# prestodb/presto

Measured on AMD Instinct MI355X. Metric: tpch_lineitem_rows_per_sec, higher is better.
Workload: dtype f64; 1 GPU; TPC-H SF100 Q1 & Q3 on 1xMI355X - one step = one Q1 pass + one Q3 pass, columns resident in HBM; query=q1+q3, rows_per_gpu=1200075804, mode=f64

## Files before the change

include/presto_gpu.h:

```cpp
#ifndef PRESTO_GPU_H
#define PRESTO_GPU_H
#include <stdint.h>

#ifdef __cplusplus
extern "C" {
#endif

#define PG_ABI_VERSION 1

typedef int32_t pg_status;
#define PG_OK 0
#define PG_ERR (-1)
const char* pg_last_error(void);

pg_status pg_device_count(int32_t* out);
pg_status pg_device_sync(void);
pg_status pg_device_malloc(int64_t bytes, void** out);
pg_status pg_device_free(void* p);
pg_status pg_memcpy_h2d(void* dst, const void* src, int64_t bytes);
pg_status pg_memcpy_d2h(void* dst, const void* src, int64_t bytes);
pg_status pg_memcpy_d2d(void* dst, const void* src, int64_t bytes);
double pg_last_hot_kernel_ms(void);
double pg_hot_max_ms(void);
void pg_hot_reset(void);
// ... 217 lines not shown
typedef enum { PG_WIN_ROW_NUMBER = 0, PG_WIN_RANK, PG_WIN_DENSE_RANK,
               PG_WIN_COUNT, PG_WIN_SUM, PG_WIN_MIN, PG_WIN_MAX,
               PG_WIN_LAG, PG_WIN_LEAD } pg_win_func;
typedef enum { PG_FRAME_RANGE_RUNNING = 0,
               PG_FRAME_ROWS_RUNNING  = 1,
               PG_FRAME_PARTITION     = 2   } pg_win_frame;
typedef struct { int32_t func;
                 int32_t col;
                 int32_t frame;
                 int32_t pad;
                 int64_t offset;
} pg_win_spec;

typedef struct {
    int32_t n_keys;
    int32_t n_partition_keys;
    int32_t key_col[PG_MAX_SORT_KEYS];
    int32_t order[PG_MAX_SORT_KEYS];
    int32_t n_emit;
    int32_t emit_cols[PG_MAX_SORT_EMIT];
    int32_t n_funcs;
    pg_win_spec funcs[PG_MAX_WIN_FUNCS];
} pg_plan_window;

#define PG_DISTINCT_MARK 0
#define PG_DISTINCT_ONLY 1

typedef struct {
    int64_t capacity_hint;
    int64_t limit;
    int32_t n_keys;
    int32_t key_col[4];
    int32_t mode;
    int32_t n_emit;
    int32_t emit_cols[16];
} pg_plan_mark_distinct;

typedef int64_t pg_op;

pg_status pg_op_create(int32_t kind, const void* plan, int64_t plan_bytes,
                       pg_op* out);
int32_t pg_op_needs_input(pg_op op);
pg_status pg_op_add_input(pg_op op, const pg_page* page);
pg_status pg_op_get_output(pg_op op, const pg_page** out);
pg_status pg_op_finish(pg_op op);
int32_t pg_op_is_finished(pg_op op);
pg_status pg_op_destroy(pg_op op);

pg_status pg_op_table(pg_op op, int64_t* out_table);
pg_status pg_op_partition_counts(pg_op op, int64_t* counts, int32_t n);

pg_status pg_table_destroy(int64_t table);
pg_status pg_table_reset_acc(int64_t table);

pg_status pg_page_serialize(const pg_page* page ,
                            void* out, int64_t cap, int64_t* out_len);
int32_t pg_abi_struct_sizes(int32_t* out, int32_t n);
int32_t pg_abi_plan_size(int32_t kind);
uint64_t pg_sortkey_u64(int32_t tag, int32_t order, uint64_t bits);

pg_status pg_page_serialize2(const pg_page* page, int32_t compress,
                             void* out, int64_t cap, int64_t* out_len);
pg_status pg_page_deserialize(const void* buf, int64_t len, pg_page* out);
pg_status pg_page_free(pg_page* page);

#ifdef __cplusplus
}
#endif
#endif
```

presto_amd/csrc/kernels.hip:

```cpp
#include <hip/hip_runtime.h>
#include <stdio.h>
#include <stdlib.h>
#include <string.h>
#include <map>
#include <vector>
#include <algorithm>
#include <type_traits>
#include <stdexcept>
#include <string>

#include "../../include/presto_gpu.h"
#include "fixed128.h"
#include "sortkey.h"

static __thread char g_err[512];
extern "C" const char* pg_last_error(void) { return g_err; }
static pg_status seterr(const char* msg)
{
    snprintf(g_err, sizeof(g_err), "%s", msg);
    return PG_ERR;
}
#define CHK(x)                                                          \
    do {                                                                \
        hipError_t e_ = (x);                                            \
// ... 1266 lines not shown
        int64_t s = (int64_t)(h & (uint64_t)mask);
        int64_t tries = 0;
        for (;;) {
            int64_t old = atomicCAS((unsigned long long*)&keys[s],
                                    (unsigned long long)TBL_EMPTY,
                                    (unsigned long long)word);
            if (old == TBL_EMPTY || old == word) {
                if (old == TBL_EMPTY) {
                    my_inserted++;
                    if (tags) tags[s] = d_tbl_tag(h);
                }
                if (pbits) break;
                if (lu_payload && dp.n >= 1)
                    ((uint8_t*)dp.ptr[0])[s] = plv;
                for (int o = lu_payload ? 1 : 0; o < dp.n; o++) {
                    const pg_col& c = pg.cols[dp.src[o]];
                    switch (dp.tag[o]) {
                        case PG_T_U8:
                            ((uint8_t*)dp.ptr[o])[s] =
                                (uint8_t)d_load_i64(c, i);
                            break;
                        case PG_T_I32:
                            ((int32_t*)dp.ptr[o])[s] =
                                (int32_t)d_load_i64(c, i);
                            break;
                        case PG_T_I64:
                            ((int64_t*)dp.ptr[o])[s] = d_load_i64(c, i);
                            break;
                        default:
                            ((double*)dp.ptr[o])[s] = d_load_f64(c, i);
                    }
                }
                break;
            }
            if (++tries > mask) {
                my_overflow++;
                break;
            }
            s = (s + 1) & mask;
        }
    }
    my_inserted = d_bfly_i64(my_inserted);
    my_overflow = d_bfly_i64(my_overflow);
    my_packerr = d_bfly_i64(my_packerr);
    if ((threadIdx.x & 63) == 0) {
        if (my_inserted) atomicAdd(inserted, (unsigned long long)my_inserted);
        if (my_overflow) atomicAdd(overflow, (unsigned long long)my_overflow);
        if (my_packerr) atomicAdd(pack_err, (unsigned long long)my_packerr);
    }
}

#define BS_R 4
#define BS_TILE (256 * BS_R)
struct staged_args {
    const int32_t* pc[2];
    int64_t pval[2];
    int32_t pop[2];
    int32_t n_preds;
    const int64_t* sk;
    const uint8_t* flags;
    int64_t nflags;
    const int64_t* lk;
    const uint8_t* lu;
    int64_t lucap;
    const int64_t* key;
    const void* pay;
    int32_t pay_tag;
    int32_t pay_pred;
    int64_t n;
};
__device__ inline bool d_cmp_i64(int32_t op, int64_t v, int64_t x)
{
    switch (op) {
        case PG_CMP_LT: return v < x;
        case PG_CMP_LE: return v <= x;
        case PG_CMP_GT: return v > x;
        case PG_CMP_GE: return v >= x;
        case PG_CMP_EQ: return v == x;
        default: return v != x;
    }
}
__device__ inline void d_bs_load_i32(const int32_t* p, int64_t base,
                                     int64_t n, bool full, int64_t* out)
{
    typedef int vi4 __attribute__((ext_vector_type(4)));
    if (full) {
        vi4 v = __builtin_nontemporal_load((const vi4*)(p + base));
#pragma unroll
        for (int j = 0; j < BS_R; j++) out[j] = v[j];
    } else {
#pragma unroll
        for (int j = 0; j < BS_R; j++)
            out[j] = base + j < n ? p[base + j] : 0;
    }
}
__device__ inline void d_bs_load_i64(const int64_t* p, int64_t base,
                                     int64_t n, bool full, int64_t* out)
{
    typedef long vl2 __attribute__((ext_vector_type(2)));
    if (full) {
#pragma unroll
        for (int j = 0; j < BS_R; j += 2) {
            vl2 v = __builtin_nontemporal_load((const vl2*)(p + base + j));
            out[j] = v[0];
            out[j + 1] = v[1];
        }
    } else {
#pragma unroll
        for (int j = 0; j < BS_R; j++)
            out[j] = base + j < n ? p[base + j] : 0;
    }
}
__device__ inline void d_bs_probe(int64_t* keys, uint8_t* tags,
                                  int64_t mask, uint64_t h, int64_t s,
                                  int64_t word, int64_t old,
                                  int64_t& my_inserted, int64_t& my_overflow)
{
    int64_t tries = 0;
    for (;;) {
        if (old == TBL_EMPTY || old == word) {
            if (old == TBL_EMPTY) {
                my_inserted++;
                if (tags) tags[s] = d_tbl_tag(h);
            }
            return;
        }
        if (++tries > mask) {
            my_overflow++;
            return;
        }
        s = (s + 1) & mask;
        old = atomicCAS((unsigned long long*)&keys[s],
                        (unsigned long long)TBL_EMPTY,
                        (unsigned long long)word);
    }
}
__global__ __launch_bounds__(256) void k_tbl_insert_staged(
    staged_args a, int32_t pbits, int64_t* keys, uint8_t* tags,
    int64_t mask, unsigned long long* inserted,
    unsigned long long* overflow, unsigned long long* pack_err,
    unsigned long long* kbits, int64_t bmax, unsigned long long* bm_err)
{
    const int64_t n = a.n;
    const int64_t n_tiles = (n + BS_TILE - 1) / BS_TILE;
    int64_t my_inserted = 0, my_overflow = 0, my_packerr = 0;
    for (int64_t tile = blockIdx.x; tile < n_tiles; tile += gridDim.x) {
        const int64_t base = tile * BS_TILE + (int64_t)threadIdx.x * BS_R;
        const bool full = base + BS_R <= n;
        int64_t pv[2][BS_R] = {}, skv[BS_R] = {}, lkv[BS_R] = {}, kv[BS_R];
        if (a.n_preds > 0) d_bs_load_i32(a.pc[0], base, n, full, pv[0]);
        if (a.n_preds > 1) d_bs_load_i32(a.pc[1], base, n, full, pv[1]);
        if (a.sk) d_bs_load_i64(a.sk, base, n, full, skv);
        if (a.lk) d_bs_load_i64(a.lk, base, n, full, lkv);
        d_bs_load_i64(a.key, base, n, full, kv);
        bool ok[BS_R];
#pragma unroll
        for (int j = 0; j < BS_R; j++) {
            ok[j] = base + j < n;
            if (a.n_preds > 0)
                ok[j] = ok[j] && d_cmp_i64(a.pop[0], pv[0][j], a.pval[0]);
            if (a.n_preds > 1)
                ok[j] = ok[j] && d_cmp_i64(a.pop[1], pv[1][j], a.pval[1]);
            if (a.lk) ok[j] = ok[j] && lkv[j] >= 1 && lkv[j] <= a.lucap;
            if (a.sk) ok[j] = ok[j] && skv[j] >= 1 && skv[j] <= a.nflags;
        }
        uint8_t fl[BS_R], plv[BS_R];
        int64_t pay[BS_R];
#pragma unroll
        for (int j = 0; j < BS_R; j++) {
            fl[j] = 1;
            plv[j] = 0;
            pay[j] = 0;
            if (!ok[j]) continue;
            if (a.sk) fl[j] = a.flags[skv[j] - 1];
            if (a.lk) plv[j] = a.lu[lkv[j] - 1];
            else if (a.pay_pred < 0) {
                if (a.pay_tag == PG_T_I32)
                    pay[j] = ((const int32_t*)a.pay)[base + j];
                else if (a.pay_tag == PG_T_U8)
                    pay[j] = ((const uint8_t*)a.pay)[base + j];
                else
                    pay[j] = ((const int64_t*)a.pay)[base + j];
            }
        }
#pragma unroll
        for (int j = 0; j < BS_R; j++) {
            ok[j] = ok[j] && fl[j] != 0;
            if (a.lk) pay[j] = plv[j];
            else if (a.pay_pred >= 0)
                pay[j] = a.pay_pred ? pv[1][j] : pv[0][j];
        }
        int64_t word[BS_R];
#pragma unroll
        for (int j = 0; j < BS_R; j++) {
            word[j] = 0;
            if (!ok[j]) continue;
            const int64_t key = kv[j];
            if (key < 0 || key >= (1ll << (63 - pbits)) || pay[j] < 0 ||
                pay[j] >= (1ll << pbits)) {
                my_packerr++;
                ok[j] = false;
                continue;
            }
            if (kbits) {
                if ((uint64_t)(key - 1) >= (uint64_t)bmax) {
                    atomicAdd(bm_err, 1ull);
                    ok[j] = false;
                    continue;
                }
                d_kbit_set(kbits, key);
            }
            word[j] = (key << pbits) | pay[j];
        }
        uint64_t h[BS_R];
        int64_t old[BS_R];
#pragma unroll
        for (int j = 0; j < BS_R; j++) {
            h[j] = pg_murmur3_finalize(pg_bigint_hash(kv[j]));
            old[j] = 0;
            if (ok[j])
                old[j] = atomicCAS(
                    (unsigned long long*)&keys[h[j] & (uint64_t)mask],
                    (unsigned long long)TBL_EMPTY,
                    (unsigned long long)word[j]);
        }
#pragma unroll
        for (int j = 0; j < BS_R; j++)
            if (ok[j])
                d_bs_probe(keys, tags, mask, h[j],
                           (int64_t)(h[j] & (uint64_t)mask), word[j], old[j],
                           my_inserted, my_overflow);
    }
    my_inserted = d_bfly_i64(my_inserted);
    my_overflow = d_bfly_i64(my_overflow);
    my_packerr = d_bfly_i64(my_packerr);
    if ((threadIdx.x & 63) == 0) {
        if (my_inserted) atomicAdd(inserted, (unsigned long long)my_inserted);
        if (my_overflow) atomicAdd(overflow, (unsigned long long)my_overflow);
        if (my_packerr) atomicAdd(pack_err, (unsigned long long)my_packerr);
    }
}

#define SCAT_TILE 8192
#define SCAT_MAXP 256

struct build_row {
    int64_t key;
    int64_t pay[4];
};

__device__ inline int d_build_eval(
    const pg_page& pg, const pg_plan_hash_build& plan,
    const int64_t* set_keys, int64_t set_mask, const int64_t* lu_keys,
    const uint8_t* lu_tags, int64_t lu_mask, int64_t lu_lmask,
    const uint8_t* lu_payload, const direct_payloads& dp, int64_t i,
    bool want_pay, build_row* out)
{
    if (!d_eval_preds<false>(pg, plan.preds, plan.n_preds, i)) return 0;
    uint8_t plv = 0;
    if (lu_payload) {
        int64_t k2 = d_load_i64(pg.cols[plan.payload_lookup_key_col], i);
        int64_t sl2;
        if (lu_keys)
            sl2 = d_tbl_find_tagged(lu_keys, lu_tags, lu_mask, lu_lmask,
                                    0, k2);
        else
            sl2 = (k2 >= 1 && k2 <= lu_mask) ? k2 - 1 : -1;
        if (sl2 < 0) return 0;
        plv = lu_payload[sl2];
        out->pay[0] = (int64_t)plv;
    }
    if (set_keys) {
        int64_t sk = d_load_i64(pg.cols[plan.semijoin_col], i);
        bool found;
        if (set_mask < 0) {
            found = sk >= 1 && sk <= -set_mask &&
                    ((const uint8_t*)set_keys)[sk - 1];
        } else {
            found = false;
            uint64_t h = pg_murmur3_finalize(pg_bigint_hash(sk));
            int64_t s = (int64_t)(h & (uint64_t)set_mask);
            for (;;) {
                int64_t k = set_keys[s];
                if (k == sk) { found = true; break; }
                if (k == TBL_EMPTY) break;
                s = (s + 1) & set_mask;
            }
        }
        if (!found) return 0;
    }
    out->key = d_load_i64(pg.cols[plan.key_col], i);
    if (want_pay) {
// ... 355 lines not shown
                nft++;
            }
        };
        for (int64_t i = base; i < lim; i++) {
            if (!d_eval_preds(pg, plan.preds, plan.n_preds, i)) continue;
            int64_t key = d_load_i64(pg.cols[plan.key_col], i);
            if (cur_slot == -2 || key != cur_key) {
                flush();
                cur_key = key;
                if (!keys)
                    cur_slot = (uint64_t)(key - 1) <= (uint64_t)mask
                                   ? key - 1
                                   : -1;
                else
                    cur_slot = kbits && !d_kbit_test(kbits, bmax, key)
                                   ? -1
                                   : d_tbl_find_tagged(keys, tags, mask,
                                                       lmask, pbits, key);
                run_dec = 0;
                run_flo = run_fhi = 0;
                run_cnt = 0;
                run_min = INT64_MAX;
            }
            if (cur_slot < 0) continue;
            pg_agg ag;
            ag.proj = plan.proj;
            ag.dec_scale = plan.dec_scale;
            int64_t ticks = d_eval_proj_dec(pg, ag, i);
            if (plan.dec_min) {
                run_min = ticks < run_min ? ticks : run_min;
            } else if (__builtin_add_overflow(run_dec, ticks, &run_dec)) {
                if (ovf) atomicAdd(ovf, 1ull);
            }
            if (!plan.dec_only && !plan.dec_min) {
                double p = d_eval_proj_f64(pg, plan.proj, i);
                uint64_t phi, plo;
                d_fx128_from_f64_ck(p, &phi, &plo, ovf + 1);
                uint64_t nlo = run_flo + plo;
                run_fhi += phi + (nlo < plo ? 1u : 0u);
                run_flo = nlo;
            }
            run_cnt++;
        }
        flush();
        if (hl.ents) {
#pragma unroll
            for (int k = 0; k < C; k++)
                d_hits_stage(hl, wbuf, &hcnt, k < nft, fts[k]);
        }
    }
    if (hl.ents && hcnt) d_hits_flush(hl, wbuf, hcnt);
}

__global__ __launch_bounds__(256)
__attribute__((amdgpu_waves_per_eu(8))) void k_probe_agg_q3(
    const int32_t* sd , int32_t pred_op,
    int32_t pred_val, const int64_t* okey, const double* ep,
    const double* dc, int64_t n, const int64_t* keys, const uint8_t* tags,
    int64_t mask, int64_t lmask, int32_t pbits,
    const unsigned long long* kbits, int64_t bmax, int32_t dec_only,
    unsigned long long* acc, int32_t aw, unsigned long long* ovf,
    hit_list hl)
{
    typedef int vi2 __attribute__((ext_vector_type(2)));
    typedef long vl2 __attribute__((ext_vector_type(2)));
    const int Q = 2;
    int64_t base0 = Q * ((int64_t)blockIdx.x * blockDim.x + threadIdx.x);
    int64_t stride = Q * (int64_t)gridDim.x * blockDim.x;
    const int lane = threadIdx.x & 63;
    __shared__ int64_t hbuf[4][WAVE];
    volatile int64_t* wbuf = hbuf[threadIdx.x >> 6];
    int hcnt = 0;
    int64_t pslot[Q];
    unsigned long long pold[Q];
#pragma unroll
    for (int j = 0; j < Q; j++) {
        pslot[j] = -1;
        pold[j] = 1;
    }
    for (int64_t base = base0; base - Q * lane < n + stride;
         base += stride) {
        int64_t k[Q];
        int32_t s[Q];
        bool sel[Q];
        if (base + Q <= n) {
            vl2 ka = __builtin_nontemporal_load((const vl2*)(okey + base));
            k[0] = ka[0]; k[1] = ka[1];
            if (sd) {
                vi2 ss = __builtin_nontemporal_load((const vi2*)(sd + base));
                s[0] = ss[0]; s[1] = ss[1];
            }
#pragma unroll
            for (int j = 0; j < Q; j++) sel[j] = true;
        } else {
#pragma unroll
            for (int j = 0; j < Q; j++) {
                sel[j] = base + j < n;
                k[j] = sel[j] ? okey[base + j] : 0;
                s[j] = sel[j] && sd ? sd[base + j] : 0;
            }
        }
        if (sd) {
#pragma unroll
            for (int j = 0; j < Q; j++)
                sel[j] = sel[j] && (pred_op == PG_CMP_GT ? s[j] > pred_val
                                                         : s[j] < pred_val);
        }
        int64_t slot[Q];
#pragma unroll
        for (int j = 0; j < Q; j++) {
            slot[j] = -1;
            if (!sel[j]) continue;
            if (kbits && !d_kbit_test(kbits, bmax, k[j])) continue;
            uint64_t h = pg_murmur3_finalize(pg_bigint_hash(k[j]));
            int64_t p = (int64_t)(h & (uint64_t)mask);
            uint8_t tg = tags ? d_tbl_tag(h) : 0;
            for (;;) {
                if (tags) {
                    uint8_t t = tags[p];
                    if (t == 0) break;
                    if (t == tg && (keys[p] >> pbits) == k[j]) {
                        slot[j] = p;
                        break;
                    }
                } else {
                    int64_t kw = keys[p];
                    if (kw == TBL_EMPTY) break;
                    if ((kw >> pbits) == k[j]) { slot[j] = p; break; }
                }
                p = d_probe_next(p, lmask);
            }
        }
        if (hl.ents) {
#pragma unroll
            for (int j = 0; j < Q; j++)
                d_hits_stage(hl, wbuf, &hcnt,
                             pslot[j] >= 0 && pold[j] == 0, pslot[j]);
        }
#pragma unroll
        for (int j = 0; j < Q; j++) {
            int64_t sl = slot[j];
            pslot[j] = sl;
            if (sl < 0) continue;
            double e = ep[base + j], d = dc[base + j];
            int64_t cents = d_round_ticks(e * 100.0);
            int64_t di = d_round_ticks(d * 100.0);
            int64_t ticks = cents * (100 - di);
            unsigned long long* s = acc + (size_t)sl * aw;
            atomicAdd(&s[0], (unsigned long long)ticks);
            if (!dec_only) {
                double pr = e * (1.0 - d);
                uint64_t phi, plo;
                d_fx128_from_f64_ck(pr, &phi, &plo, ovf + 1);
                unsigned long long old = atomicAdd(&s[1], plo);
                atomicAdd(&s[2], phi + (old > ~plo ? 1ull : 0ull));
            }
            pold[j] = atomicAdd(&s[aw - 1], 1ull);
        }
    }
    if (hl.ents && hcnt) d_hits_flush(hl, wbuf, hcnt);
}

__global__ __launch_bounds__(256) void k_probe_agg_pay(
    pg_page pg, pg_plan_lookup_join plan, const int64_t* keys1,
    const uint8_t* tags1, const int32_t* head1, int64_t mask1,
    int64_t lmask1, const unsigned long long* kbits1, int64_t bmax1,
    const int64_t* pay1, const int64_t* keys2,
    const uint8_t* tags2, int64_t mask2, int64_t lmask2,
    unsigned long long* acc2, int32_t aw, unsigned long long* ovf)
{
    int64_t i = (int64_t)blockIdx.x * blockDim.x + threadIdx.x;
    int64_t stride = (int64_t)gridDim.x * blockDim.x;
    for (; i < pg.n_rows; i += stride) {
        if (!d_eval_preds(pg, plan.preds, plan.n_preds, i)) continue;
        int64_t key = d_load_i64(pg.cols[plan.key_col], i);
        if (kbits1 && !d_kbit_test(kbits1, bmax1, key)) continue;
        int64_t s1 = d_tbl_find_tagged(keys1, tags1, mask1, lmask1, 0,
                                       key);
        if (s1 < 0) continue;
        int64_t r = head1 ? (int64_t)head1[s1] : s1;
        if (r < 0) continue;
        int64_t g = pay1[r];
        int64_t s2 =
// ... 3303 lines not shown
        if (plan.range_group) {
            if (plan.capacity_hint <= 0)
                throw std::runtime_error(
                    "range_group needs capacity_hint = max key");
            t->range_group = true;
            t->slot_payloads = true;
            t->cap = plan.capacity_hint;
            t->mask = t->cap - 1;
            t->local_mask = t->mask;
            return;
        }
        if (plan.dense_array) {
            if (plan.n_payload != 1 && !plan.key_set_only)
                throw std::runtime_error(
                    "dense_array needs one u8 payload (or key_set_only)");
            t->dense = true;
            t->cap = plan.capacity_hint;
            t->payload.emplace_back();
            t->ptag.push_back(PG_T_U8);
            t->dense_alloc_pending = true;
            if (plan.key_set_only) {
                t->payload.back().alloc((size_t)t->cap);
                t->payload.back().zero();
                t->dense_alloc_pending = false;
            }
            return;
        }
        if (plan.agg_table) {
            t->slot_payloads = true;
            if (plan.pack_bits) {
                if (plan.n_payload != 1 || plan.pack_bits < 1 ||
                    plan.pack_bits > 32)
                    throw std::runtime_error(
                        "pack_bits needs exactly one payload and "
                        "1..32 bits");
                t->pack_bits = plan.pack_bits;
            }
            int64_t mult10 = plan.fill_x10 >= 11 ? plan.fill_x10 : 20;
            if (const char* em = getenv("PG_CAP_X10"))
                if (atoi(em) >= 11) mult10 = atoi(em);
            int64_t cap = next_pow2(plan.capacity_hint * mult10 / 10 + 16);
            t->cap = cap;
            t->mask = cap - 1;
            t->local_mask = cap - 1;
            t->keys.alloc((size_t)cap * 8);
            int64_t part_min = 512ll << 20;
            if (const char* ep = getenv("PG_PART_MIN_SLOTS"))
                if (atoll(ep) > 0) part_min = atoll(ep);
            part = cap >= part_min;
            staged = true;
            if (const char* es = getenv("PG_BUILD_STAGED"))
                staged = atoi(es) != 0;
            bool always_hit = plan.fill_x10 >= 11 && plan.fill_x10 < 20;
            if (!always_hit && (part || cap >= (64ll << 20))) {
                t->tags.alloc((size_t)cap);
                if (!part) t->tags.zero();
            }
            counters.alloc(40);
            counters.zero();
            if (plan.bitmap_max_key > 0) {
                t->bmax = plan.bitmap_max_key;
                t->kbits.alloc((size_t)((t->bmax >> 6) + 1) * 8);
                t->kbits.zero();
            }
            if (part) {
                P = 256;
                while (cap / P < (64ll << 10)) P >>= 1;
                int64_t slot_bytes = 8 + (t->tags.p ? 1 : 0) +
                                     8ll * plan.n_payload;
                int64_t region_bytes = cap / P * slot_bytes;
                Kact = (int32_t)((128ll << 20) / region_bytes);
                if (Kact < 1) Kact = 1;
                if (Kact > P) Kact = P;
                const char* ek = getenv("PG_PART_K");
                if (ek && atoi(ek) > 0) {
                    Kact = atoi(ek);
                    if (Kact > P) Kact = P;
                }
                int64_t cap_p = cap / P;
                capp_bits = 0;
                while ((1ll << capp_bits) < cap_p) capp_bits++;
                t->local_mask = cap_p - 1;
                int32_t r_words = 1 + plan.n_payload;
                stage.alloc((size_t)cap * r_words * 8);
                cursorb.alloc((size_t)P * 8);
                cursorb.zero();
                barb.alloc(8);
                barb.zero();
            } else {
                hipLaunchKernelGGL(k_tbl_init, dim3(1024), dim3(256), 0,
                                   g_stream, (int64_t*)t->keys.p, nullptr,
                                   cap);
            }
            for (int i = 0; i < plan.n_payload; i++) {
                t->payload.emplace_back();
                t->ptag.push_back(-1);
                t->payload.back().alloc(
                    plan.pack_bits ? 1 : (size_t)cap * 8);
            }
            return;
        }
        cap_rows = plan.capacity_hint > 16 ? plan.capacity_hint : 16;
        t->n_keys = plan.n_keys;
        t->key_rows.alloc((size_t)cap_rows * 8 * key_words());
        if (plan.n_keys) t->knull.alloc((size_t)cap_rows);
        for (int i = 0; i < plan.n_payload; i++) {
            t->payload.emplace_back();
// ... 194 lines not shown
                    plan.key_set_only
                        ? nullptr
                        : (const uint8_t*)
                              sp.pg.cols[plan.payload_col[0]].data,
                    (uint8_t*)t->payload[0].p, t->cap);
            CHKV(hipStreamSynchronize(g_stream));
            return;
        }
        if (plan.agg_table) {
            const Table* semi = semi_table();
            const Table* lu = nullptr;
            if (plan.payload_lookup_table > 0) {
                std::lock_guard<std::mutex> lk(g_mu);
                auto it = g_tables.find(plan.payload_lookup_table);
                if (it == g_tables.end() ||
                    !(it->second->slot_payloads || it->second->dense) ||
                    it->second->ptag.empty() ||
                    it->second->ptag[0] != PG_T_U8)
                    throw std::runtime_error(
                        "payload_lookup_table must be an agg_table or "
                        "dense_array with a u8 payload");
                lu = it->second.get();
            }
            direct_payloads dp{};
            dp.n = plan.n_payload;
            for (int o = 0; o < dp.n; o++) {
                dp.ptr[o] = t->payload[o].p;
                dp.tag[o] = lu && o == 0 ? PG_T_U8 : t->ptag[o];
                dp.src[o] = plan.payload_col[o];
            }
            if (part) {
                hot_begin();
                hipLaunchKernelGGL(
                    k_part_scatter, dim3(2048), dim3(256), 0, g_stream,
                    sp.pg, plan, set_ptr(semi), set_mask_of(semi),
                    lu && !lu->dense ? (const int64_t*)lu->keys.p
                                     : nullptr,
                    lu && !lu->dense ? (const uint8_t*)lu->tags.p
                                     : nullptr,
                    lu ? (lu->dense ? lu->cap : lu->mask) : 0,
                    lu ? (lu->dense ? lu->cap : lu->local_mask) : 0,
                    lu ? (const uint8_t*)lu->payload[0].p : nullptr, dp,
                    t->mask, capp_bits, P, (int64_t*)stage.p,
                    (unsigned long long*)cursorb.p, t->cap / P,
                    1 + plan.n_payload,
                    (unsigned long long*)counters.p + 2);
                hot_end();
                CHKV(hipStreamSynchronize(g_stream));
                return;
            }
            staged_args sa;
            if (staged_fit(sp.pg, semi, lu, &sa)) {
                int64_t tiles = (sa.n + BS_TILE - 1) / BS_TILE;
                int grid = (int)(tiles < 4096 ? (tiles > 0 ? tiles : 1)
                                              : 4096);
                hot_begin();
                hipLaunchKernelGGL(
                    k_tbl_insert_staged, dim3(grid), dim3(256), 0, g_stream,
                    sa, plan.pack_bits, (int64_t*)t->keys.p,
                    (uint8_t*)t->tags.p, t->mask,
                    (unsigned long long*)counters.p,
                    (unsigned long long*)counters.p + 1,
                    (unsigned long long*)counters.p + 3,
                    (unsigned long long*)t->kbits.p, t->bmax,
                    (unsigned long long*)counters.p + 4);
                hot_end();
                g_build_staged_launches++;
                CHKV(hipStreamSynchronize(g_stream));
                return;
            }
            hot_begin();
            hipLaunchKernelGGL(k_tbl_insert_direct, dim3(4096), dim3(256),
                               0, g_stream, sp.pg, plan, set_ptr(semi),
                               set_mask_of(semi),
                               lu && !lu->dense
                                   ? (const int64_t*)lu->keys.p
                                   : nullptr,
                               lu && !lu->dense
                                   ? (const uint8_t*)lu->tags.p
                                   : nullptr,
                               lu ? (lu->dense ? lu->cap : lu->mask) : 0,
                               lu ? (lu->dense ? lu->cap : lu->local_mask)
                                  : 0,
                               lu ? (const uint8_t*)lu->payload[0].p
                                  : nullptr,
                               (int64_t*)t->keys.p,
                               (uint8_t*)t->tags.p, dp, t->mask,
                               (unsigned long long*)counters.p,
                               (unsigned long long*)counters.p + 1,
                               (unsigned long long*)counters.p + 3,
                               (unsigned long long*)t->kbits.p, t->bmax,
                               (unsigned long long*)counters.p + 4);
            hot_end();
            CHKV(hipStreamSynchronize(g_stream));
            return;
        }
        pg_plan_filter_project fp{};
        fp.n_preds = plan.n_preds;
        memcpy(fp.preds, plan.preds, sizeof(fp.preds));
        fp.n_proj = 1 + plan.n_payload;
        fp.proj[0].kind = PG_PROJ_IDENT;
        fp.proj[0].a = plan.key_col;
        for (int i = 0; i < plan.n_payload; i++) {
            fp.proj[1 + i].kind = PG_PROJ_IDENT;
            fp.proj[1 + i].a = plan.payload_col[i];
        }
        const Table* semi = nullptr;
        if (plan.semijoin_table >= 0) {
            std::lock_guard<std::mutex> lk(g_mu);
            auto it = g_tables.find(plan.semijoin_table);
            if (it == g_tables.end())
// ... 555 lines not shown
                               (const uint8_t*)t->tags.p,
                               (const int32_t*)t->head.p, t->mask,
                               t->local_mask,
                               (const unsigned long long*)t->kbits.p, t->bmax,
                               (const int64_t*)t->payload[0].p,
                               (const int64_t*)t2->keys.p,
                               (const uint8_t*)t2->tags.p, t2->mask,
                               t2->local_mask,
                               (unsigned long long*)t2->acc.p,
                               t2->acc_words,
                               (unsigned long long*)ovf.p);
            hot_end();
            CHKV(hipStreamSynchronize(g_stream));
            return;
        }
        if (plan.mode == 1 && plan.n_aggs > 0) {
            hot_begin();
            hipLaunchKernelGGL(k_probe_agg_multi, dim3(4096), dim3(256), 0,
                               g_stream, sp.pg, plan,
                               (const int64_t*)t->keys.p,
                               (const uint8_t*)t->tags.p, t->mask,
                               t->local_mask, t->pack_bits,
                               (const unsigned long long*)t->kbits.p, t->bmax,
                               (unsigned long long*)t->acc_multi.p,
                               (unsigned long long*)ovf.p);
            hot_end();
            CHKV(hipStreamSynchronize(g_stream));
            return;
        }
        if (plan.mode == 1) {
            bool spec = plan.proj.kind == PG_PROJ_DISC_PRICE &&
                        !plan.dec_min &&
                        sp.pg.cols[plan.key_col].tag == PG_T_I64 &&
                        sp.pg.cols[plan.proj.a].tag == PG_T_F64 &&
                        sp.pg.cols[plan.proj.b].tag == PG_T_F64 &&
                        plan.dec_scale == 4 && plan.n_preds <= 1 &&
                        !((uintptr_t)sp.pg.cols[plan.key_col].data & 15) &&
                        !((uintptr_t)sp.pg.cols[plan.proj.a].data & 15) &&
                        !((uintptr_t)sp.pg.cols[plan.proj.b].data & 15);
            if (plan.n_preds == 1) {
                const pg_pred& pr = plan.preds[0];
                spec = spec && pr.rhs_col == 0 &&
                       sp.pg.cols[pr.col].tag == PG_T_I32 &&
                       (pr.op == PG_CMP_GT || pr.op == PG_CMP_LT) &&
                       !((uintptr_t)sp.pg.cols[pr.col].data & 7) &&
                       !sp.pg.cols[pr.col].null_mask;
            }
            spec = spec && !sp.pg.cols[plan.key_col].null_mask &&
                   !sp.pg.cols[plan.proj.a].null_mask &&
                   !sp.pg.cols[plan.proj.b].null_mask;
            hot_begin();
            if (spec) {
                const pg_pred& pr = plan.preds[0];
                hipLaunchKernelGGL(
                    k_probe_agg_q3, dim3(4096), dim3(256), 0, g_stream,
                    plan.n_preds
                        ? (const int32_t*)sp.pg.cols[pr.col].data
                        : nullptr,
                    plan.n_preds ? pr.op : 0,
                    plan.n_preds ? (int32_t)pr.ival : 0,
                    (const int64_t*)sp.pg.cols[plan.key_col].data,
                    (const double*)sp.pg.cols[plan.proj.a].data,
                    (const double*)sp.pg.cols[plan.proj.b].data,
                    sp.pg.n_rows, (const int64_t*)t->keys.p,
                    (const uint8_t*)t->tags.p, t->mask, t->local_mask,
                    t->pack_bits, (const unsigned long long*)t->kbits.p, t->bmax, plan.dec_only,
                    (unsigned long long*)t->acc.p, t->acc_words,
                    (unsigned long long*)ovf.p, hits_arg(t));
            } else {
                hipLaunchKernelGGL(k_probe_agg, dim3(4096), dim3(256), 0,
                                   g_stream, sp.pg, plan,
                                   (const int64_t*)t->keys.p,
                                   (const uint8_t*)t->tags.p, t->mask,
                                   t->local_mask, t->pack_bits,
                                   (const unsigned long long*)t->kbits.p, t->bmax,
                                   (unsigned long long*)t->acc.p,
                                   t->acc_words,
                                   (unsigned long long*)ovf.p, hits_arg(t));
            }
            hot_end();
            if (t->list_ok)
                CHKV(hipMemcpyAsync(&t->hits_n_host, t->hits_n.p, 8,
                                    hipMemcpyDeviceToHost, g_stream));
            CHKV(hipStreamSynchronize(g_stream));
            return;
        }
        int64_t n = sp.pg.n_rows;
        const bool typed_cols = outer() || plan.n_keys;
        if (typed_cols && probe_tags.empty())
            for (int o = 0; o < plan.n_emit; o++)
                probe_tags.push_back(
                    sp.pg.cols[plan.emit_probe_cols[o]].tag);
        if (n == 0) {
            OutPage op;
            op.pg.n_rows = 0;
            op.pg.n_cols = plan.n_emit + (int32_t)t->payload.size();
            for (int c = 0; c < op.pg.n_cols; c++) {
                op.pg.cols[c].tag = PG_T_I64;
                if (typed_cols)
                    op.pg.cols[c].tag =
                        c < plan.n_emit ? probe_tags[c]
                                        : payload_tag(t, c - plan.n_emit);
                op.pg.cols[c].on_device = 1;
                op.pg.cols[c].data = nullptr;
            }
            outq.push_back(std::move(op));
            return;
        }
// ... 1773 lines not shown
}
extern "C" pg_status pg_op_finish(pg_op h)
{
    auto op = find_op(h);
    if (!op) return seterr("bad op handle");
    if (op->finished) return PG_OK;
    try {
        op->finish();
        op->finished = true;
        return PG_OK;
    } catch (std::exception& e) {
        return seterr(e.what());
    }
}
extern "C" int32_t pg_op_is_finished(pg_op h)
{
    auto op = find_op(h);
    return op && op->finished && op->outq.empty() ? 1 : 0;
}
extern "C" pg_status pg_op_destroy(pg_op h)
{
    std::lock_guard<std::mutex> lk(g_mu);
    g_ops.erase(h);
    return PG_OK;
}
extern "C" pg_status pg_op_table(pg_op h, int64_t* out)
{
    auto op = find_op(h);
    if (!op) return seterr("bad op handle");
    int64_t t = op->table_handle();
    if (t < 0) return seterr("op has no table (finish the build first)");
    *out = t;
    return PG_OK;
}
extern "C" pg_status pg_op_partition_counts(pg_op h, int64_t* counts,
                                            int32_t n)
{
    auto op = find_op(h);
    if (!op) return seterr("bad op handle");
    try {
        op->partition_counts(counts, n);
        return PG_OK;
    } catch (std::exception& e) {
        return seterr(e.what());
    }
}
extern "C" pg_status pg_table_destroy(int64_t t)
{
    std::lock_guard<std::mutex> lk(g_mu);
    g_tables.erase(t);
    return PG_OK;
}

extern "C" pg_status pg_table_reset_acc(int64_t t)
{
    try {
        Table* tbl;
        {
            std::lock_guard<std::mutex> lk(g_mu);
            auto it = g_tables.find(t);
            if (it == g_tables.end())
                return seterr("pg_table_reset_acc: table not found");
            tbl = it->second.get();
        }
        if (tbl->acc.p) {
            CHK(hipMemsetAsync(tbl->acc.p, 0, tbl->acc.sz, g_stream));
            hits_restart(tbl);
        }
        if (tbl->acc_multi.p)
            CHK(hipMemsetAsync(tbl->acc_multi.p, 0, tbl->acc_multi.sz,
                               g_stream));
        CHK(hipStreamSynchronize(g_stream));
        return PG_OK;
    } catch (const std::exception& e) {
        return seterr(e.what());
    }
}

namespace {

static uint32_t crc32_tab_[256];
static bool crc32_init_ = false;
static uint32_t pg_crc32(uint32_t crc, const uint8_t* p, size_t n)
{
    if (!crc32_init_) {
        for (uint32_t i = 0; i < 256; i++) {
            uint32_t c = i;
            for (int k = 0; k < 8; k++)
                c = (c & 1) ? 0xEDB88320u ^ (c >> 1) : c >> 1;
            crc32_tab_[i] = c;
        }
        crc32_init_ = true;
    }
    crc = ~crc;
    for (size_t i = 0; i < n; i++)
        crc = crc32_tab_[(crc ^ p[i]) & 0xff] ^ (crc >> 8);
    return ~crc;
}

struct ByteWriter {
    uint8_t* p;
    int64_t cap, off = 0;
    bool ok = true;
    void bytes(const void* src, int64_t n)
    {
        if (off + n > cap) { ok = false; return; }
// ... 580 lines not shown
```

presto_amd/engine.py:

```python
import contextlib
import ctypes as C
import pathlib

import numpy as np

_HERE = pathlib.Path(__file__).resolve().parent
_SO = _HERE / "libpresto_gpu.so"

T_U8, T_I32, T_I64, T_F64, T_VARBIN, T_I128 = 0, 1, 2, 3, 4, 5
(CMP_LT, CMP_LE, CMP_GT, CMP_GE, CMP_EQ, CMP_NE, CMP_CONTAINS,
 CMP_PREFIX, CMP_CONTAINS2, CMP_NOT_CONTAINS2, CMP_IS_NULL,
 CMP_IS_NOT_NULL) = range(12)
JOIN_INNER, JOIN_PROBE_OUTER, JOIN_LOOKUP_OUTER, JOIN_FULL_OUTER = 0, 4, 5, 6
(PROJ_IDENT, PROJ_DISC_PRICE, PROJ_CHARGE, PROJ_MUL, PROJ_DIV,
 PROJ_KEYSHL, PROJ_SHR, PROJ_SUBDIV, PROJ_KEYSHL_DIV) = range(9)
(AGG_COUNT, AGG_SUM_F64, AGG_SUM_DEC, AGG_SUM_I64,
 AGG_MIN, AGG_MAX) = range(6)
(OP_FILTER_PROJECT, OP_HASH_AGG_SMALL, OP_HASH_BUILD, OP_LOOKUP_JOIN,
 OP_TOPN, OP_PARTITION, OP_GROUPBY_MULTI, OP_ORDER_BY) = range(1, 9)
OP_WINDOW = 10
OP_MARK_DISTINCT = 12
DISTINCT_MARK, DISTINCT_ONLY = 0, 1
(SORT_ASC_NULLS_FIRST, SORT_ASC_NULLS_LAST, SORT_DESC_NULLS_FIRST,
 SORT_DESC_NULLS_LAST) = range(4)
# ... 104 lines not shown
                ("order", C.c_int32 * 4), ("n_emit", C.c_int32),
                ("emit_cols", C.c_int32 * 16), ("limit", C.c_int64)]


class WinSpec(C.Structure):
    _fields_ = [("func", C.c_int32), ("col", C.c_int32),
                ("frame", C.c_int32), ("pad", C.c_int32),
                ("offset", C.c_int64)]


class PlanWindow(C.Structure):
    _fields_ = [("n_keys", C.c_int32), ("n_partition_keys", C.c_int32),
                ("key_col", C.c_int32 * 4), ("order", C.c_int32 * 4),
                ("n_emit", C.c_int32), ("emit_cols", C.c_int32 * 16),
                ("n_funcs", C.c_int32), ("funcs", WinSpec * 8)]


class PlanMarkDistinct(C.Structure):
    _fields_ = [("capacity_hint", C.c_int64), ("limit", C.c_int64),
                ("n_keys", C.c_int32), ("key_col", C.c_int32 * 4),
                ("mode", C.c_int32), ("n_emit", C.c_int32),
                ("emit_cols", C.c_int32 * 16)]


_ABI_STRUCTS = (PgCol, PgPage, Pred, Proj, Agg, PlanFilterProject,
                PlanHashAggSmall, PlanHashBuild, PlanLookupJoin, PlanGroupBy,
                PlanTopN, PlanPartition)
_ABI_PLANS = ((PlanOrderBy, OP_ORDER_BY), (PlanWindow, OP_WINDOW),
              (PlanMarkDistinct, OP_MARK_DISTINCT))


class _Lib:
    def __init__(self):
        if not _SO.exists():
            raise RuntimeError(
                f"{_SO} not built — run __graft_entry__.build() first "
                "(the product HIP library is required; no CPU fallback)")
        self.c = C.CDLL(str(_SO))
        self.c.pg_last_error.restype = C.c_char_p
        self.c.pg_op_create.argtypes = [C.c_int32, C.c_void_p, C.c_int64,
                                        C.POINTER(C.c_int64)]
        self.c.pg_op_add_input.argtypes = [C.c_int64, C.POINTER(PgPage)]
        self.c.pg_op_get_output.argtypes = [C.c_int64,
                                            C.POINTER(C.POINTER(PgPage))]
        for f in ("pg_op_finish", "pg_op_destroy", "pg_op_needs_input",
                  "pg_op_is_finished"):
            getattr(self.c, f).argtypes = [C.c_int64]
        self.c.pg_op_table.argtypes = [C.c_int64, C.POINTER(C.c_int64)]
        self.c.pg_op_partition_counts.argtypes = [C.c_int64,
                                                  C.POINTER(C.c_int64),
                                                  C.c_int32]
        self.c.pg_table_destroy.argtypes = [C.c_int64]
        self.c.pg_table_reset_acc.argtypes = [C.c_int64]
        self.c.pg_memcpy_d2h.argtypes = [C.c_void_p, C.c_void_p, C.c_int64]
        self.c.pg_memcpy_d2d.argtypes = [C.c_void_p, C.c_void_p, C.c_int64]
        self.c.pg_memcpy_h2d.argtypes = [C.c_void_p, C.c_void_p, C.c_int64]
        self.c.pg_device_sync.argtypes = []
        self.c.pg_abi_plan_size.argtypes = [C.c_int32]
        self.c.pg_abi_plan_size.restype = C.c_int32
        self.c.pg_sortkey_u64.argtypes = [C.c_int32, C.c_int32, C.c_uint64]
        self.c.pg_sortkey_u64.restype = C.c_uint64
        self.c.pg_multikey_probe_pages.argtypes = []
        self.c.pg_multikey_probe_pages.restype = C.c_int64
        self.c.pg_abi_struct_sizes.argtypes = [C.POINTER(C.c_int32),
                                               C.c_int32]
        self.c.pg_abi_struct_sizes.restype = C.c_int32
        self._check_struct_sizes()

    def _check_struct_sizes(self):
        n = self.c.pg_abi_struct_sizes(None, 0)
        sizes = (C.c_int32 * n)()
        self.c.pg_abi_struct_sizes(sizes, n)
        bad = [f"{cls.__name__}: ctypes {C.sizeof(cls)}, library {sz}"
               for cls, sz in zip(_ABI_STRUCTS, sizes)
               if C.sizeof(cls) != sz]
        for cls, kind in _ABI_PLANS:
            sz = self.c.pg_abi_plan_size(kind)
            if C.sizeof(cls) != sz:
                bad.append(f"{cls.__name__}: ctypes {C.sizeof(cls)}, "
                           f"library {sz}")
        if n < len(_ABI_STRUCTS):
            bad.append(f"pg_abi_struct_sizes reports {n} structs, the "
                       f"binding mirrors {len(_ABI_STRUCTS)}")
        if bad:
            raise RuntimeError(
                f"{_SO} does not match the ctypes mirrors of "
                "include/presto_gpu.h (rebuild the library): "
                + "; ".join(bad))

    def err(self):
        return (self.c.pg_last_error() or b"").decode()

    def check(self, st, what):
        if st != 0:
            raise RuntimeError(f"{what}: {self.err()}")


_lib = None


def lib():
    global _lib
    if _lib is None:
        _lib = _Lib()
    return _lib

# ... 337 lines not shown
```

Measured before the change: 136.5 billion rows/s.

## Specialize staged build and Q3 probe kernels via templates; skip tags with exact bitmap

Templates the staged hash-build kernel on predicate count, semijoin/lookup presence and payload type, so runtime branches become compile-time ones and loads are vectorized on full tiles. Templates the Q3 probe kernel on key-bitmap and tag presence, and hoists the bitmap test and the first tag/key loads ahead of the probe loop so memory latency overlaps across the unrolled rows. Tag-array allocation is skipped when an exact key bitmap already filters probes, which removes tag memory traffic but makes probes compare full keys. Grid sizes can now be overridden through environment variables, and a small API reports tag bytes.

```diff
diff --git a/include/presto_gpu.h b/include/presto_gpu.h
--- a/include/presto_gpu.h
+++ b/include/presto_gpu.h
@@ -293,6 +293,7 @@
 
 pg_status pg_table_destroy(int64_t table);
 pg_status pg_table_reset_acc(int64_t table);
+int64_t pg_table_tag_bytes(int64_t table);
 
 pg_status pg_page_serialize(const pg_page* page ,
                             void* out, int64_t cap, int64_t* out_len);
diff --git a/presto_amd/csrc/kernels.hip b/presto_amd/csrc/kernels.hip
--- a/presto_amd/csrc/kernels.hip
+++ b/presto_amd/csrc/kernels.hip
@@ -1342,6 +1342,14 @@
 
 #define BS_R 4
 #define BS_TILE (256 * BS_R)
+#define BS_GRID 4096
+enum {
+    BS_PAY_PRED = 0,
+    BS_PAY_LOOKUP,
+    BS_PAY_I32,
+    BS_PAY_U8,
+    BS_PAY_I64
+};
 struct staged_args {
     const int32_t* pc[2];
     int64_t pval[2];
@@ -1370,36 +1378,29 @@
         default: return v != x;
     }
 }
-__device__ inline void d_bs_load_i32(const int32_t* p, int64_t base,
-                                     int64_t n, bool full, int64_t* out)
+__device__ inline void d_bs_vload_i32(const int32_t* p, int32_t* out)
 {
     typedef int vi4 __attribute__((ext_vector_type(4)));
-    if (full) {
-        vi4 v = __builtin_nontemporal_load((const vi4*)(p + base));
+    vi4 v = __builtin_nontemporal_load((const vi4*)p);
 #pragma unroll
-        for (int j = 0; j < BS_R; j++) out[j] = v[j];
-    } else {
+    for (int j = 0; j < BS_R; j++) out[j] = v[j];
+}
+__device__ inline void d_bs_vload_i64(const int64_t* p, int64_t* out)
+{
+    typedef long vl2 __attribute__((ext_vector_type(2)));
 #pragma unroll
-        for (int j = 0; j < BS_R; j++)
-            out[j] = base + j < n ? p[base + j] : 0;
-    }
-}
-__device__ inline void d_bs_load_i64(const int64_t* p, int64_t base,
-                                     int64_t n, bool full, int64_t* out)
-{
-    typedef long vl2 __attribute__((ext_vector_type(2)));
-    if (full) {
-#pragma unroll
-        for (int j = 0; j < BS_R; j += 2) {
-            vl2 v = __builtin_nontemporal_load((const vl2*)(p + base + j));
-            out[j] = v[0];
-            out[j + 1] = v[1];
-        }
-    } else {
-#pragma unroll
-        for (int j = 0; j < BS_R; j++)
-            out[j] = base + j < n ? p[base + j] : 0;
-    }
+    for (int j = 0; j < BS_R; j += 2) {
+        vl2 v = __builtin_nontemporal_load((const vl2*)(p + j));
+        out[j] = v[0];
+        out[j + 1] = v[1];
+    }
+}
+template <int PAY>
+__device__ inline int64_t d_bs_pay(const void* p, int64_t i)
+{
+    if constexpr (PAY == BS_PAY_I32) return ((const int32_t*)p)[i];
+    else if constexpr (PAY == BS_PAY_U8) return ((const uint8_t*)p)[i];
+    else return ((const int64_t*)p)[i];
 }
 __device__ inline void d_bs_probe(int64_t* keys, uint8_t* tags,
                                   int64_t mask, uint64_t h, int64_t s,
@@ -1425,59 +1426,69 @@
                         (unsigned long long)word);
     }
 }
+template <int NP, bool SK, bool LK, int PAY>
 __global__ __launch_bounds__(256) void k_tbl_insert_staged(
     staged_args a, int32_t pbits, int64_t* keys, uint8_t* tags,
     int64_t mask, unsigned long long* inserted,
     unsigned long long* overflow, unsigned long long* pack_err,
     unsigned long long* kbits, int64_t bmax, unsigned long long* bm_err)
 {
+    constexpr bool OWN_PAY = PAY >= BS_PAY_I32;
     const int64_t n = a.n;
     const int64_t n_tiles = (n + BS_TILE - 1) / BS_TILE;
     int64_t my_inserted = 0, my_overflow = 0, my_packerr = 0;
     for (int64_t tile = blockIdx.x; tile < n_tiles; tile += gridDim.x) {
         const int64_t base = tile * BS_TILE + (int64_t)threadIdx.x * BS_R;
-        const bool full = base + BS_R <= n;
-        int64_t pv[2][BS_R] = {}, skv[BS_R] = {}, lkv[BS_R] = {}, kv[BS_R];
-        if (a.n_preds > 0) d_bs_load_i32(a.pc[0], base, n, full, pv[0]);
-        if (a.n_preds > 1) d_bs_load_i32(a.pc[1], base, n, full, pv[1]);
-        if (a.sk) d_bs_load_i64(a.sk, base, n, full, skv);
-        if (a.lk) d_bs_load_i64(a.lk, base, n, full, lkv);
-        d_bs_load_i64(a.key, base, n, full, kv);
+        int32_t pv[2][BS_R] = {};
+        int64_t skv[BS_R] = {}, lkv[BS_R] = {}, kv[BS_R], pay[BS_R] = {};
+        if (base + BS_R <= n) {
+            if constexpr (NP > 0) d_bs_vload_i32(a.pc[0] + base, pv[0]);
+            if constexpr (NP > 1) d_bs_vload_i32(a.pc[1] + base, pv[1]);
+            if constexpr (SK) d_bs_vload_i64(a.sk + base, skv);
+            if constexpr (LK) d_bs_vload_i64(a.lk + base, lkv);
+            d_bs_vload_i64(a.key + base, kv);
+            if constexpr (OWN_PAY) {
+#pragma unroll
+                for (int j = 0; j < BS_R; j++)
+                    pay[j] = d_bs_pay<PAY>(a.pay, base + j);
+            }
+        } else {
+#pragma unroll
+            for (int j = 0; j < BS_R; j++) {
+                const bool in = base + j < n;
+                if constexpr (NP > 0) pv[0][j] = in ? a.pc[0][base + j] : 0;
+                if constexpr (NP > 1) pv[1][j] = in ? a.pc[1][base + j] : 0;
+                if constexpr (SK) skv[j] = in ? a.sk[base + j] : 0;
+                if constexpr (LK) lkv[j] = in ? a.lk[base + j] : 0;
+                kv[j] = in ? a.key[base + j] : 0;
+                if constexpr (OWN_PAY)
+                    pay[j] = in ? d_bs_pay<PAY>(a.pay, base + j) : 0;
+            }
+        }
         bool ok[BS_R];
 #pragma unroll
         for (int j = 0; j < BS_R; j++) {
             ok[j] = base + j < n;
-            if (a.n_preds > 0)
+            if constexpr (NP > 0)
                 ok[j] = ok[j] && d_cmp_i64(a.pop[0], pv[0][j], a.pval[0]);
-            if (a.n_preds > 1)
+            if constexpr (NP > 1)
                 ok[j] = ok[j] && d_cmp_i64(a.pop[1], pv[1][j], a.pval[1]);
-            if (a.lk) ok[j] = ok[j] && lkv[j] >= 1 && lkv[j] <= a.lucap;
-            if (a.sk) ok[j] = ok[j] && skv[j] >= 1 && skv[j] <= a.nflags;
+            if constexpr (LK)
+                ok[j] = ok[j] && lkv[j] >= 1 && lkv[j] <= a.lucap;
+            if constexpr (SK)
+                ok[j] = ok[j] && skv[j] >= 1 && skv[j] <= a.nflags;
         }
         uint8_t fl[BS_R], plv[BS_R];
-        int64_t pay[BS_R];
 #pragma unroll
         for (int j = 0; j < BS_R; j++) {
-            fl[j] = 1;
-            plv[j] = 0;
-            pay[j] = 0;
-            if (!ok[j]) continue;
-            if (a.sk) fl[j] = a.flags[skv[j] - 1];
-            if (a.lk) plv[j] = a.lu[lkv[j] - 1];
-            else if (a.pay_pred < 0) {
-                if (a.pay_tag == PG_T_I32)
-                    pay[j] = ((const int32_t*)a.pay)[base + j];
-                else if (a.pay_tag == PG_T_U8)
-                    pay[j] = ((const uint8_t*)a.pay)[base + j];
-                else
-                    pay[j] = ((const int64_t*)a.pay)[base + j];
-            }
+            if constexpr (SK) fl[j] = a.flags[ok[j] ? skv[j] - 1 : 0];
+            if constexpr (LK) plv[j] = a.lu[ok[j] ? lkv[j] - 1 : 0];
         }
 #pragma unroll
         for (int j = 0; j < BS_R; j++) {
-            ok[j] = ok[j] && fl[j] != 0;
-            if (a.lk) pay[j] = plv[j];
-            else if (a.pay_pred >= 0)
+            if constexpr (SK) ok[j] = ok[j] && fl[j] != 0;
+            if constexpr (LK) pay[j] = plv[j];
+            else if constexpr (PAY == BS_PAY_PRED)
                 pay[j] = a.pay_pred ? pv[1][j] : pv[0][j];
         }
         int64_t word[BS_R];
@@ -1528,6 +1539,36 @@
         if (my_inserted) atomicAdd(inserted, (unsigned long long)my_inserted);
         if (my_overflow) atomicAdd(overflow, (unsigned long long)my_overflow);
         if (my_packerr) atomicAdd(pack_err, (unsigned long long)my_packerr);
+    }
+}
+typedef void (*staged_fn)(staged_args, int32_t, int64_t*, uint8_t*, int64_t,
+                          unsigned long long*, unsigned long long*,
+                          unsigned long long*, unsigned long long*, int64_t,
+                          unsigned long long*);
+template <int NP, bool SK>
+static staged_fn bs_pick_pay(const staged_args& a)
+{
+    if (a.lk) return k_tbl_insert_staged<NP, SK, true, BS_PAY_LOOKUP>;
+    if (a.pay_pred >= 0)
+        return k_tbl_insert_staged<NP, SK, false, BS_PAY_PRED>;
+    switch (a.pay_tag) {
+        case PG_T_I32:
+            return k_tbl_insert_staged<NP, SK, false, BS_PAY_I32>;
+        case PG_T_U8:
+            return k_tbl_insert_staged<NP, SK, false, BS_PAY_U8>;
+        default:
+            return k_tbl_insert_staged<NP, SK, false, BS_PAY_I64>;
+    }
+}
+static staged_fn bs_pick(const staged_args& a)
+{
+    switch (a.n_preds) {
+        case 0:
+            return a.sk ? bs_pick_pay<0, true>(a) : bs_pick_pay<0, false>(a);
+        case 1:
+            return a.sk ? bs_pick_pay<1, true>(a) : bs_pick_pay<1, false>(a);
+        default:
+            return a.sk ? bs_pick_pay<2, true>(a) : bs_pick_pay<2, false>(a);
     }
 }
 
@@ -1989,6 +2030,9 @@
     if (hl.ents && hcnt) d_hits_flush(hl, wbuf, hcnt);
 }
 
+#define PQ3_Q 2
+#define PQ3_GRID 4096
+template <bool KB, bool TAGS>
 __global__ __launch_bounds__(256)
 __attribute__((amdgpu_waves_per_eu(8))) void k_probe_agg_q3(
     const int32_t* sd , int32_t pred_op,
@@ -2001,7 +2045,7 @@
 {
     typedef int vi2 __attribute__((ext_vector_type(2)));
     typedef long vl2 __attribute__((ext_vector_type(2)));
-    const int Q = 2;
+    const int Q = PQ3_Q;
     int64_t base0 = Q * ((int64_t)blockIdx.x * blockDim.x + threadIdx.x);
     int64_t stride = Q * (int64_t)gridDim.x * blockDim.x;
     const int lane = threadIdx.x & 63;
@@ -2018,14 +2062,22 @@
     for (int64_t base = base0; base - Q * lane < n + stride;
          base += stride) {
         int64_t k[Q];
-        int32_t s[Q];
+        int32_t s[Q] = {};
         bool sel[Q];
         if (base + Q <= n) {
-            vl2 ka = __builtin_nontemporal_load((const vl2*)(okey + base));
-            k[0] = ka[0]; k[1] = ka[1];
+#pragma unroll
+            for (int j = 0; j < Q; j += 2) {
+                vl2 ka = __builtin_nontemporal_load(
+                    (const vl2*)(okey + base + j));
+                k[j] = ka[0]; k[j + 1] = ka[1];
+            }
             if (sd) {
-                vi2 ss = __builtin_nontemporal_load((const vi2*)(sd + base));
-                s[0] = ss[0]; s[1] = ss[1];
+#pragma unroll
+                for (int j = 0; j < Q; j += 2) {
+                    vi2 ss = __builtin_nontemporal_load(
+                        (const vi2*)(sd + base + j));
+                    s[j] = ss[0]; s[j + 1] = ss[1];
+                }
             }
 #pragma unroll
             for (int j = 0; j < Q; j++) sel[j] = true;
@@ -2043,29 +2095,47 @@
                 sel[j] = sel[j] && (pred_op == PG_CMP_GT ? s[j] > pred_val
                                                          : s[j] < pred_val);
         }
+        if constexpr (KB) {
+            unsigned long long w[Q];
+#pragma unroll
+            for (int j = 0; j < Q; j++) {
+                sel[j] = sel[j] && (uint64_t)(k[j] - 1) < (uint64_t)bmax;
+                w[j] = kbits[sel[j] ? (uint64_t)k[j] >> 6 : 0];
+            }
+#pragma unroll
+            for (int j = 0; j < Q; j++)
+                sel[j] = sel[j] && ((w[j] >> (k[j] & 63)) & 1);
+        }
+        constexpr bool KEY_WITH_TAG = KB || !TAGS;
+        int64_t p[Q], kw[Q];
+        uint8_t tg[Q], t[Q];
+#pragma unroll
+        for (int j = 0; j < Q; j++) {
+            uint64_t h = pg_murmur3_finalize(pg_bigint_hash(k[j]));
+            p[j] = sel[j] ? (int64_t)(h & (uint64_t)mask) : 0;
+            tg[j] = d_tbl_tag(h);
+            t[j] = 0;
+            kw[j] = 0;
+            if constexpr (TAGS) t[j] = tags[p[j]];
+            if constexpr (KEY_WITH_TAG) kw[j] = keys[p[j]];
+        }
         int64_t slot[Q];
 #pragma unroll
         for (int j = 0; j < Q; j++) {
             slot[j] = -1;
             if (!sel[j]) continue;
-            if (kbits && !d_kbit_test(kbits, bmax, k[j])) continue;
-            uint64_t h = pg_murmur3_finalize(pg_bigint_hash(k[j]));
-            int64_t p = (int64_t)(h & (uint64_t)mask);
-            uint8_t tg = tags ? d_tbl_tag(h) : 0;
             for (;;) {
-                if (tags) {
-                    uint8_t t = tags[p];
-                    if (t == 0) break;
-                    if (t == tg && (keys[p] >> pbits) == k[j]) {
-                        slot[j] = p;
+                if (TAGS ? t[j] == 0 : kw[j] == TBL_EMPTY) break;
+                if (!TAGS || t[j] == tg[j]) {
+                    if constexpr (!KEY_WITH_TAG) kw[j] = keys[p[j]];
+                    if ((kw[j] >> pbits) == k[j]) {
+                        slot[j] = p[j];
                         break;
                     }
-                } else {
-                    int64_t kw = keys[p];
-                    if (kw == TBL_EMPTY) break;
-                    if ((kw >> pbits) == k[j]) { slot[j] = p; break; }
                 }
-                p = d_probe_next(p, lmask);
+                p[j] = d_probe_next(p[j], lmask);
+                if constexpr (TAGS) t[j] = tags[p[j]];
+                if constexpr (KEY_WITH_TAG) kw[j] = keys[p[j]];
             }
         }
         if (hl.ents) {
@@ -5475,7 +5545,9 @@
             if (const char* es = getenv("PG_BUILD_STAGED"))
                 staged = atoi(es) != 0;
             bool always_hit = plan.fill_x10 >= 11 && plan.fill_x10 < 20;
-            if (!always_hit && (part || cap >= (64ll << 20))) {
+            bool exact_bitmap = !part && plan.bitmap_max_key > 0;
+            if (!always_hit && !exact_bitmap &&
+                (part || cap >= (64ll << 20))) {
                 t->tags.alloc((size_t)cap);
                 if (!part) t->tags.zero();
             }
@@ -5776,11 +5848,18 @@
             staged_args sa;
             if (staged_fit(sp.pg, semi, lu, &sa)) {
                 int64_t tiles = (sa.n + BS_TILE - 1) / BS_TILE;
-                int grid = (int)(tiles < 4096 ? (tiles > 0 ? tiles : 1)
-                                              : 4096);
+                int64_t cap_grid = BS_GRID;
+                if (const char* eg = getenv("PG_STAGED_GRID"))
+                    if (atoi(eg) > 0) cap_grid = atoi(eg);
+                int grid = (int)(tiles < cap_grid ? (tiles > 0 ? tiles : 1)
+                                                  : cap_grid);
+                if (sa.sk && sa.nflags <= 0)
+                    sa.flags = (const uint8_t*)counters.p;
+                if (sa.lk && sa.lucap <= 0)
+                    sa.lu = (const uint8_t*)counters.p;
                 hot_begin();
                 hipLaunchKernelGGL(
-                    k_tbl_insert_staged, dim3(grid), dim3(256), 0, g_stream,
+                    bs_pick(sa), dim3(grid), dim3(256), 0, g_stream,
                     sa, plan.pack_bits, (int64_t*)t->keys.p,
                     (uint8_t*)t->tags.p, t->mask,
                     (unsigned long long*)counters.p,
@@ -6442,8 +6521,17 @@
             hot_begin();
             if (spec) {
                 const pg_pred& pr = plan.preds[0];
+                auto kern =
+                    t->kbits.p
+                        ? (t->tags.p ? k_probe_agg_q3<true, true>
+                                     : k_probe_agg_q3<true, false>)
+                        : (t->tags.p ? k_probe_agg_q3<false, true>
+                                     : k_probe_agg_q3<false, false>);
+                int grid = PQ3_GRID;
+                if (const char* eg = getenv("PG_PROBE_GRID"))
+                    if (atoi(eg) > 0) grid = atoi(eg);
                 hipLaunchKernelGGL(
-                    k_probe_agg_q3, dim3(4096), dim3(256), 0, g_stream,
+                    kern, dim3(grid), dim3(256), 0, g_stream,
                     plan.n_preds
                         ? (const int32_t*)sp.pg.cols[pr.col].data
                         : nullptr,
@@ -8323,6 +8411,14 @@
     return PG_OK;
 }
 
+extern "C" int64_t pg_table_tag_bytes(int64_t t)
+{
+    std::lock_guard<std::mutex> lk(g_mu);
+    auto it = g_tables.find(t);
+    if (it == g_tables.end()) return 0;
+    return it->second->tags.p ? (int64_t)it->second->tags.sz : 0;
+}
+
 extern "C" pg_status pg_table_reset_acc(int64_t t)
 {
     try {
diff --git a/presto_amd/engine.py b/presto_amd/engine.py
--- a/presto_amd/engine.py
+++ b/presto_amd/engine.py
@@ -180,6 +180,8 @@
                                                   C.c_int32]
         self.c.pg_table_destroy.argtypes = [C.c_int64]
         self.c.pg_table_reset_acc.argtypes = [C.c_int64]
+        self.c.pg_table_tag_bytes.argtypes = [C.c_int64]
+        self.c.pg_table_tag_bytes.restype = C.c_int64
         self.c.pg_memcpy_d2h.argtypes = [C.c_void_p, C.c_void_p, C.c_int64]
         self.c.pg_memcpy_d2d.argtypes = [C.c_void_p, C.c_void_p, C.c_int64]
         self.c.pg_memcpy_h2d.argtypes = [C.c_void_p, C.c_void_p, C.c_int64]
```

After: 142.0 billion rows/s (median of 6 runs). +4.0%, better.
